# hypermagik/srsRAN-5G

Measured on AMD Instinct MI355X. Metric: PDSCH+PUSCH slots/sec (100MHz 4x4) + LDPC info-bits/s at 1/2/4/8 GPU, higher is better.
Workload: dtype int8/bf16/f32; 1 GPU

## Files before the change

srsran-5g_amd/csrc/capi_pdsch_mod.cpp:

```cpp
#include "capi_internal.h"
#include <algorithm>
#include <cmath>
#include <cstring>
#include <vector>

using namespace srsgpu;

static_assert(sizeof(srsgpu_pdsch_mod_config) == 168, "srsgpu_pdsch_mod_config layout (mirrored by srsgpu.PdschModConfig)");

static_assert(sizeof(srsgpu_pdsch_dmrs_config) == 152, "srsgpu_pdsch_dmrs_config layout (mirrored by srsgpu)");

struct srsgpu_pdsch_dmrs_plan {
  srsgpu_context* ctx      = nullptr;
  device_buffer<dmrs_job> d_jobs;
  device_buffer<uint32_t> d_seq;
  int             nof_jobs = 0;
  int             max_pilots = 0;
};

struct srsgpu_pdsch_modulator_plan {
  srsgpu_context* ctx        = nullptr;
  device_buffer<mod_desc>  d_desc;
  device_buffer<uint16_t>  d_sc_map;
  device_buffer<float>     d_prg_w;
// ... 216 lines not shown
    if (c.nof_symbols < 1 || c.start_symbol + c.nof_symbols > 14) {
      return fail(SRSGPU_ERR_INVALID_ARG, "tx %u: time allocation [%u, %u) exceeds the slot", t, c.start_symbol,
                  c.start_symbol + c.nof_symbols);
    }
    if ((c.dmrs_type != 1 && c.dmrs_type != 2) || c.nof_cdm_groups_without_data < 1 ||
        c.nof_cdm_groups_without_data > (c.dmrs_type == 1 ? 2 : 3)) {
      return fail(SRSGPU_ERR_INVALID_ARG, "tx %u: invalid DM-RS type %u / CDM groups without data %u", t,
                  c.dmrs_type, c.nof_cdm_groups_without_data);
    }
    const bool general = x != nullptr && (x->crb_mask != nullptr || x->nof_reserved > 0 || x->prg_size > 0);
    if (c.n_id > 1023 || c.bwp_size_rb < 1 || c.bwp_start_rb + c.bwp_size_rb > grid_nof_prb ||
        (!general && (c.nof_rb < 1 || c.rb_start + c.nof_rb > c.bwp_size_rb))) {
      return fail(SRSGPU_ERR_INVALID_ARG, "tx %u: allocation outside the BWP or the grid, or n_id > 1023", t);
    }
    if (x != nullptr && ((x->nof_reserved > 0 && x->reserved == nullptr) ||
                         (x->prg_size > 0 && (x->prg_weights == nullptr || x->nof_prg == 0 ||
                                              static_cast<uint32_t>(x->prg_size) * x->nof_prg < grid_nof_prb)))) {
      return fail(SRSGPU_ERR_INVALID_ARG, "tx %u: invalid allocation extension (reserved patterns / PRG weights)", t);
    }
    if (c.cw_offset % 4 != 0) {
      return fail(SRSGPU_ERR_INVALID_ARG, "tx %u: codeword offset not a multiple of 4", t);
    }
    mod_desc d{};
    unsigned nd = 0;
    for (unsigned k = 0; k < 12; ++k) {
      const unsigned group = (c.dmrs_type == 2) ? (k % 6) / 2 : k % 2;
      if (group >= c.nof_cdm_groups_without_data) {
        d.dmrs_lut |= static_cast<uint64_t>(k) << (4 * nd);
        ++nd;
      }
    }
    d.nd_dmrs = static_cast<uint8_t>(nd);
    uint32_t nre = 0;
    d.sc_map     = NO_SC_MAP;
    if (general) {
      std::vector<uint8_t> crbs(grid_nof_prb, 0);
      for (unsigned rb = 0; rb < grid_nof_prb; ++rb) {
        crbs[rb] = (x->crb_mask != nullptr) ? x->crb_mask[rb]
                                            : (rb >= c.bwp_start_rb + c.rb_start &&
                                               rb < static_cast<unsigned>(c.bwp_start_rb + c.rb_start + c.nof_rb));
      }
      enumerate_data_res(grid_nof_prb, crbs.data(), c.start_symbol, c.nof_symbols, c.dmrs_symbol_mask, c.dmrs_type,
                         c.nof_cdm_groups_without_data, c.bwp_start_rb, c.bwp_start_rb + c.bwp_size_rb, x->reserved,
                         x->nof_reserved, sc_tx, d.sym_cum);
      nre      = static_cast<uint32_t>(sc_tx.size());
      d.sc_map = static_cast<uint32_t>(sc_map.size());
      sc_map.insert(sc_map.end(), sc_tx.begin(), sc_tx.end());
    } else {
      for (unsigned l = 0; l < 14; ++l) {
        d.sym_cum[l] = static_cast<uint16_t>(nre);
        if (l >= c.start_symbol && l < static_cast<unsigned>(c.start_symbol + c.nof_symbols)) {
          nre += (((c.dmrs_symbol_mask >> l) & 1u) ? nd : 12u) * c.nof_rb;
        }
      }
      d.sym_cum[14] = static_cast<uint16_t>(nre);
      d.sym_cum[15] = static_cast<uint16_t>(nre);
    }
    const uint64_t need = static_cast<uint64_t>(nre) * c.nof_layers * qm;
    if (nre == 0 || need != c.nof_bits || c.nof_bits > MOD_MAX_BITS) {
      return fail(SRSGPU_ERR_INVALID_ARG, "tx %u: codeword of %u bits for %u data REs x %u layers x Qm %u", t,
                  c.nof_bits, nre, c.nof_layers, qm);
    }
    d.cw_word_offset = c.cw_offset / 4;
    d.nof_bits       = c.nof_bits;
    d.c_init         = (static_cast<uint32_t>(c.rnti) << 15) + c.n_id;
    d.port_stride    = 14u * nsc;
    d.nsc            = nsc;
    d.grid_base      = c.grid_index * grid_nof_ports * 14u * nsc + (general ? 0u : (c.bwp_start_rb + c.rb_start) * 12u);
    d.dmrs_mask      = c.dmrs_symbol_mask;
    d.qm             = static_cast<uint8_t>(qm);
    d.L              = c.nof_layers;
    d.P              = c.nof_ports;
    float amp = modulation_amplitude(qm);
    if (std::isnormal(c.scaling)) {
      amp *= c.scaling;
    }
    for (int p = 0; p < 4; ++p) {
      for (int l = 0; l < 4; ++l) {
        const bool used = p < c.nof_ports && l < c.nof_layers;
        d.w[p][l][0]    = used ? c.precoding[p][l][0] * amp : 0.f;
        d.w[p][l][1]    = used ? c.precoding[p][l][1] * amp : 0.f;
      }
    }
    d.prg_sc = 0;
    if (x != nullptr && x->prg_size > 0) {
      d.prg_sc = static_cast<uint16_t>(x->prg_size * 12u);
      d.prg_w  = static_cast<uint32_t>(prg_w.size());
      for (unsigned g = 0; g < x->nof_prg; ++g) {
        for (int p = 0; p < 4; ++p) {
          for (int l = 0; l < 4; ++l) {
            const bool   used = p < c.nof_ports && l < c.nof_layers;
            const float* src  = x->prg_weights + ((static_cast<size_t>(g) * c.nof_ports + p) * c.nof_layers + l) * 2;
            prg_w.push_back(used ? src[0] * amp : 0.f);
            prg_w.push_back(used ? src[1] * amp : 0.f);
          }
        }
      }
    }
    descs[t]              = d;
    const uint32_t Lq     = static_cast<uint32_t>(c.nof_layers) * qm;
    const uint32_t nwords = (c.nof_bits + 31) / 32;
    for (uint32_t w0 = 0; w0 < nwords; w0 += MOD_CHUNK_WORDS) {
      const uint32_t b0 = w0 * 32, b1 = b0 + MOD_CHUNK_WORDS * 32;
      mod_chunk      ch{};
      ch.tx       = t;
      ch.word0    = w0;
      ch.re_begin = (b0 + Lq - 1) / Lq;
      ch.re_end   = std::min(nre, (b1 + Lq - 1) / Lq);
      if (ch.re_end > ch.re_begin) {
        chunks.push_back(ch);
      }
    }
  }
  std::vector<uint32_t> c_inits(descs.size()), nwords(descs.size());
  for (size_t t = 0; t < descs.size(); ++t) {
    c_inits[t] = descs[t].c_init;
    nwords[t]  = (descs[t].nof_bits + 31u) / 32u;
  }
  const std::vector<uint32_t> seq_off = gold_sequence_offsets(nwords);
  for (size_t t = 0; t < descs.size(); ++t) {
    descs[t].seq_word_offset = seq_off[t];
  }
  plan_ptr<srsgpu_pdsch_modulator_plan> plan(new srsgpu_pdsch_modulator_plan());
  plan->ctx        = ctx;
  plan->nof_chunks = static_cast<int>(chunks.size());
  if (!chunks.empty()) {
    if (build_gold_sequences(ctx, c_inits, nwords, seq_off, plan->d_seq) != SRSGPU_OK) {
      return SRSGPU_ERR_HIP;
    }
    if (!plan->d_desc.upload(descs) || !plan->d_chunks.upload(chunks) || !plan->d_sc_map.upload(sc_map) ||
        !plan->d_prg_w.upload(prg_w)) {
      return fail(SRSGPU_ERR_HIP, "failed to upload modulator descriptors");
    }
  }
  *plan_out = plan.release();
  return SRSGPU_OK;
}

int srsgpu_pdsch_modulator_plan_execute(const srsgpu_pdsch_modulator_plan* plan,
                                        const uint8_t*                     d_codewords,
                                        uint32_t*                          d_grids,
                                        void*                              stream)
{
  if (plan == nullptr || d_codewords == nullptr || d_grids == nullptr) {
    return fail(SRSGPU_ERR_INVALID_ARG, "null argument");
  }
  launch_pdsch_modulate(plan->d_desc.get(), plan->d_sc_map.get(), plan->d_prg_w.get(), plan->d_chunks.get(),
                        plan->nof_chunks, reinterpret_cast<const uint32_t*>(d_codewords), d_grids, plan->d_seq.get(),
                        static_cast<hipStream_t>(stream));
  HIP_TRY(hipGetLastError());
  return SRSGPU_OK;
}

void srsgpu_pdsch_modulator_plan_destroy(srsgpu_pdsch_modulator_plan* plan)
{
  if (plan == nullptr) {
    return;
  }
  delete plan;
}

int srsgpu_pdsch_dmrs_plan_create(srsgpu_context*                 ctx,
                                  const srsgpu_pdsch_dmrs_config* cfgs,
                                  uint32_t                        nof_tx,
                                  uint32_t                        grid_nof_prb,
                                  uint32_t                        grid_nof_ports,
                                  srsgpu_pdsch_dmrs_plan**        plan_out)
{
// ... 132 lines not shown
```

srsran-5g_amd/csrc/crc_device.h:

```cpp
#pragma once

#include "common.h"

namespace srsgpu {

__device__ __forceinline__ uint32_t gf2_mulmod(uint32_t a, uint32_t b, uint32_t g, int order)
{
  const uint32_t high = 1u << order;
  uint32_t       r    = 0;
  for (int i = order - 1; i >= 0; --i) {
    r <<= 1;
    if (r & high) {
      r ^= g;
    }
    if ((b >> i) & 1u) {
      r ^= a;
    }
  }
  return r;
}

__device__ inline uint32_t block_crc_bytes(const uint8_t* data, int n, int order, uint32_t g, uint32_t* table,
                                           uint32_t* part)
{
// ... 24 lines not shown
  }
  __syncthreads();
  uint32_t f = 1u;
  {
    uint32_t base = 2u;
    uint32_t e    = 8u * static_cast<uint32_t>(cs);
    while (e) {
      if (e & 1u) {
        f = gf2_mulmod(f, base, g, order);
      }
      base = gf2_mulmod(base, base, g, order);
      e >>= 1;
    }
  }
  for (int step = 1; step < 256; step <<= 1) {
    if (in && (threadIdx.x % (2 * step)) == 0) {
      part[threadIdx.x] = gf2_mulmod(part[threadIdx.x], f, g, order) ^ part[threadIdx.x + step];
    }
    f = gf2_mulmod(f, f, g, order);
    __syncthreads();
  }
  const uint32_t crc = part[0];
  __syncthreads();
  return crc;
}

__device__ inline uint32_t block_crc_table(const uint8_t* data, int nbytes, const uint32_t* P, uint32_t* red)
{
  uint32_t acc = 0;
  for (int j = threadIdx.x; j < nbytes; j += blockDim.x) {
    const uint32_t byte = data[j];
    const uint4*   p4   = reinterpret_cast<const uint4*>(P + 8 * j);
    const uint4    a    = p4[0];
    const uint4    b    = p4[1];
    acc ^= (byte & 0x80u) ? a.x : 0u;
    acc ^= (byte & 0x40u) ? a.y : 0u;
    acc ^= (byte & 0x20u) ? a.z : 0u;
    acc ^= (byte & 0x10u) ? a.w : 0u;
    acc ^= (byte & 0x08u) ? b.x : 0u;
    acc ^= (byte & 0x04u) ? b.y : 0u;
    acc ^= (byte & 0x02u) ? b.z : 0u;
    acc ^= (byte & 0x01u) ? b.w : 0u;
  }
  acc = wave_xor(acc);
  if ((threadIdx.x % WAVE) == 0) {
    red[threadIdx.x / WAVE] = acc;
  }
  __syncthreads();
  uint32_t crc = 0;
  for (int w = 0; w < static_cast<int>(blockDim.x / WAVE); ++w) {
    crc ^= red[w];
  }
  __syncthreads();
  return crc;
}

__device__ inline void crc_byte_lut(uint32_t* lut, int order, uint32_t g)
{
  const uint32_t mask = (1u << order) - 1u;
  for (uint32_t t = threadIdx.x; t < 256u; t += blockDim.x) {
    uint32_t r = t << (order - 8);
    for (int k = 0; k < 8; ++k) {
      r <<= 1;
      if (r & (1u << order)) {
        r ^= g;
      }
    }
    lut[t] = r & mask;
  }
  __syncthreads();
}

__device__ __forceinline__ uint32_t gf2_mulmod(uint32_t r, uint32_t M, int order, uint32_t g)
{
  uint32_t acc = 0;
#pragma unroll
  for (int b = 23; b >= 0; --b) {
    acc = (acc << 1) ^ (((acc >> (order - 1)) & 1u) ? g : 0u);
    acc ^= ((M >> b) & 1u) ? r : 0u;
  }
  return acc;
}

__device__ __forceinline__ uint32_t crc_step4(uint32_t r, uint32_t m, int order, const uint32_t* T)
{
  const uint32_t u = (r << (32 - order)) ^ m;
  return T[u & 0xffu] ^ T[256u + ((u >> 8) & 0xffu)] ^ T[512u + ((u >> 16) & 0xffu)] ^ T[768u + (u >> 24)];
}

template <int CS, typename Data>
__device__ inline uint32_t block_crc_slice4(Data data, int nbytes, const uint32_t* P, int order, uint32_t g,
                                            const uint32_t* T, uint32_t* red, bool have_m0 = false, uint32_t m0 = 0)
{
  static_assert(CS % 4 == 0, "whole words per chunk");
  const uint32_t mask = (1u << order) - 1u;
  const int      L    = 8 * nbytes;
  const int      nch  = (nbytes + CS - 1) / CS;
  const int      c0   = static_cast<int>(threadIdx.x);
  uint32_t       acc  = 0;
  for (int c = c0; c < nch; c += blockDim.x) {
    const int      b0 = c * CS;
    const int      b1 = min(b0 + CS, nbytes);
    const int      j  = 8 * b1 + order - 1;
    const uint32_t M  = (have_m0 && c == c0) ? m0 : ((j < L) ? P[j] : (1u << (order + L - 1 - j)));
    uint32_t       byte[CS];
#pragma unroll
    for (int k = 0; k < CS; ++k) {
      byte[k] = (b0 + k < b1) ? static_cast<uint32_t>(data(b0 + k)) : 0u;
    }
    uint32_t rem = 0;
#pragma unroll
    for (int w = 0; w < CS / 4; ++w) {
      const int k = 4 * w;
      if (b0 + k + 4 <= b1) {
        rem = crc_step4(rem, (byte[k] << 24) | (byte[k + 1] << 16) | (byte[k + 2] << 8) | byte[k + 3], order, T);
      } else {
#pragma unroll
        for (int q = 0; q < 4; ++q) {
          if (b0 + k + q < b1) {
            rem = ((rem << 8) ^ T[((rem >> (order - 8)) ^ byte[k + q]) & 0xffu]) & mask;
          }
        }
      }
    }
    acc ^= gf2_mulmod(rem, M, order, g);
  }
  acc = wave_xor(acc);
  if ((threadIdx.x % WAVE) == 0) {
    red[threadIdx.x / WAVE] = acc;
  }
  __syncthreads();
  uint32_t crc = 0;
  for (int w = 0; w < static_cast<int>((blockDim.x + WAVE - 1) / WAVE); ++w) {
    crc ^= red[w];
  }
  __syncthreads();
  return crc;
}

template <int CS>
__device__ __forceinline__ uint32_t crc_chunk_power(int c, int nbytes, const uint32_t* P, int order)
{
  const int L  = 8 * nbytes;
  const int b1 = min((c + 1) * CS, nbytes);
  const int j  = 8 * b1 + order - 1;
  return (j < L) ? P[j] : (1u << (order + L - 1 - j));
}

template <int CS, typename Data>
__device__ inline uint32_t block_crc_chunks(Data data, int nbytes, const uint32_t* P, int order, uint32_t g,
                                            const uint32_t* lut, uint32_t* red, int begin = 0, int end = -1,
                                            bool have_m0 = false, uint32_t m0 = 0)
{
  const uint32_t mask = (1u << order) - 1u;
  const int      L    = 8 * nbytes;
  const int      nch  = ((end < 0 ? nbytes : end) + CS - 1) / CS;
  const int      c0   = begin / CS + static_cast<int>(threadIdx.x);
  uint32_t       acc  = 0;
  for (int c = c0; c < nch; c += blockDim.x) {
    const int b0  = c * CS;
    const int b1  = min(b0 + CS, nbytes);
    const int j   = 8 * b1 + order - 1;
    const uint32_t M = (have_m0 && c == c0) ? m0 : ((j < L) ? P[j] : (1u << (order + L - 1 - j)));
    uint32_t byte[CS];
#pragma unroll
    for (int k = 0; k < CS; ++k) {
      byte[k] = (b0 + k < b1) ? static_cast<uint32_t>(data(b0 + k)) : 0u;
    }
    uint32_t rem = 0;
#pragma unroll
    for (int k = 0; k < CS; ++k) {
      if (b0 + k < b1) {
        rem = ((rem << 8) ^ lut[((rem >> (order - 8)) ^ byte[k]) & 0xffu]) & mask;
      }
    }
    acc ^= gf2_mulmod(rem, M, order, g);
  }
  acc = wave_xor(acc);
  if ((threadIdx.x % WAVE) == 0) {
    red[threadIdx.x / WAVE] = acc;
  }
  __syncthreads();
  uint32_t crc = 0;
  for (int w = 0; w < static_cast<int>((blockDim.x + WAVE - 1) / WAVE); ++w) {
    crc ^= red[w];
  }
  __syncthreads();
  return crc;
}

}
```

srsran-5g_amd/csrc/ldpc_encoder.hip:

```cpp
#include "common.h"
#include "crc_device.h"
#include "ldpc_base_graphs.h"
#include "srsgpu_internal.h"

namespace srsgpu {
namespace {

#ifdef ENC_PROFILE
constexpr int ENC_PROF_CBS   = 8192;
constexpr int ENC_PROF_SLOTS = 16;
__device__ uint64_t g_enc_prof[ENC_PROF_CBS * ENC_PROF_SLOTS];
#define ENC_PROF(slot, value)                                                                                          \
  do {                                                                                                                 \
    if (threadIdx.x == 0 && blockIdx.x < ENC_PROF_CBS) {                                                               \
      g_enc_prof[blockIdx.x * ENC_PROF_SLOTS + (slot)] = (value);                                                      \
    }                                                                                                                  \
  } while (0)
#else
#define ENC_PROF(slot, value)                                                                                          \
  do {                                                                                                                 \
  } while (0)
#endif
#define ENC_STAMP(slot) ENC_PROF(slot, __builtin_amdgcn_s_memtime())

// ... 493 lines not shown
  tcd.order       = d.tb_crc_len;
  tcd.poly        = (d.tb_crc_len == 24) ? 0x1864cfbu : 0x11021u;
  tcd.table       = d.tb_crc_table;
  constexpr int TCS   = 16;
  const bool    tfast = carrier && tcd.nbytes <= 2u * TCS * PK_THREADS && ((tcd.byte_offset | tcd.nbytes) & 3u) == 0u;
  uint32_t      tw[2][TCS / 4];
  uint32_t      tm[2] = {0u, 0u};
  if (tfast) {
    const uint32_t* tbw = reinterpret_cast<const uint32_t*>(tbs + tcd.byte_offset);
    const int       nw  = static_cast<int>(tcd.nbytes / 4u);
#pragma unroll
    for (int h = 0; h < 2; ++h) {
      const int c = tid + h * PK_THREADS;
#pragma unroll
      for (int q = 0; q < TCS / 4; ++q) {
        const int w = c * (TCS / 4) + q;
        tw[h][q]    = (w < nw) ? tbw[w] : 0u;
      }
      if (c * TCS < static_cast<int>(tcd.nbytes)) {
        tm[h] = crc_chunk_power<TCS>(c, static_cast<int>(tcd.nbytes), crc_tables + tcd.table,
                                     static_cast<int>(tcd.order));
      }
    }
  }
  constexpr int TW = CRC_SLICE_WORDS / PK_THREADS;
  if (has_cbc) {
    const uint32_t* src = crc_slice + CRC_SLICE_24B * CRC_SLICE_WORDS;
    uint32_t        t[TW];
#pragma unroll
    for (int q = 0; q < TW; ++q) {
      t[q] = src[tid + q * PK_THREADS];
    }
#pragma unroll
    for (int q = 0; q < TW; ++q) {
      t4b[tid + q * PK_THREADS] = t[q];
    }
  }
  if (carrier) {
    const uint32_t* src = crc_slice + (tcd.order == 24 ? CRC_SLICE_24A : CRC_SLICE_16) * CRC_SLICE_WORDS;
    uint32_t        t[TW];
#pragma unroll
    for (int q = 0; q < TW; ++q) {
      t[q] = src[tid + q * PK_THREADS];
    }
#pragma unroll
    for (int q = 0; q < TW; ++q) {
      uni[tid + q * PK_THREADS] = t[q];
    }
  }
  for (int m = tid; m <= G::M; m += PK_THREADS) {
    row_start[m] = static_cast<uint16_t>(G::rs(m));
  }
#pragma unroll
  for (int r = 0; r < MB; ++r) {
    const int q = tid + r * PK_THREADS;
    if (q < nkb) {
      const uint32_t p = d.tb_bit_offset + 8u * static_cast<uint32_t>(q);
      uint32_t       b = byte[r];
      if (q < nd8 && p >= d.tb_bits) {
        b = (tb_crc >> (d.tb_crc_len - 8u - (p - d.tb_bits))) & 0xffu;
      }
      msg[q] = static_cast<uint8_t>(b);
    }
  }
  __syncthreads();
  if (tfast) {
    const int order  = static_cast<int>(tcd.order);
    const int nb     = static_cast<int>(tcd.nbytes);
    uint32_t  rem[2] = {0u, 0u};
#pragma unroll
    for (int q = 0; q < TCS / 4; ++q) {
#pragma unroll
      for (int h = 0; h < 2; ++h) {
        const int c = tid + h * PK_THREADS;
        if (c * TCS + 4 * q < nb) {
          rem[h] = crc_step4(rem[h], __builtin_bswap32(tw[h][q]), order, t4t);
        }
      }
    }
    uint32_t acc = 0;
#pragma unroll
    for (int h = 0; h < 2; ++h) {
      if ((tid + h * PK_THREADS) * TCS < nb) {
        acc ^= gf2_mulmod(rem[h], tm[h], order, tcd.poly);
      }
    }
    acc = wave_xor(acc);
    if ((tid % WAVE) == 0) {
      red[tid / WAVE] = acc;
    }
    __syncthreads();
#pragma unroll
    for (int w = 0; w < PK_THREADS / WAVE; ++w) {
      tb_crc ^= red[w];
    }
  } else if (carrier) {
    const uint8_t* tbp = tbs + tcd.byte_offset;
    tb_crc = block_crc_slice4<16>([tbp](int i) { return tbp[i]; }, static_cast<int>(tcd.nbytes),
                                  crc_tables + tcd.table, static_cast<int>(tcd.order), tcd.poly, t4t, red);
  }
  ENC_STAMP(1);
  if (carrier) {
    const int qc = static_cast<int>(d.tb_bits - min(d.tb_bit_offset, d.tb_bits)) / 8;
    if (tid < nd8 - qc) {
      const uint32_t p = d.tb_bit_offset + 8u * static_cast<uint32_t>(qc + tid);
      msg[qc + tid]    = static_cast<uint8_t>((tb_crc >> (d.tb_crc_len - 8u - (p - d.tb_bits))) & 0xffu);
    }
  }
  ENC_STAMP(2);
  if (has_cbc) {
    if (carrier) {
      __syncthreads();
    }
    const uint32_t crc = block_crc_slice4<CB_CS>([](int q) { return msg[q]; }, cb_bytes, crc_tables + d.crc_table, 24,
                                                 0x1800063u, t4b, red, pre_m, m0);
    if (tid < 3) {
      msg[d.used / 8 + tid] = static_cast<uint8_t>(crc >> (16 - 8 * tid));
    }
  }
  __syncthreads();
  ENC_STAMP(3);
  const uint32_t* msg32 = reinterpret_cast<const uint32_t*>(msg);
  for (int q = tid; q < K * W; q += PK_THREADS) {
    cw[q] = bytes_bitrev(msg32[q]);
  }
  if (tid < 4 * WMAX) {
    lam[tid] = 0u;
  }
#pragma unroll
  for (int r = 0; r < NEL; ++r) {
    if (tid + r * PK_THREADS < G::NE) {
      edge[tid + r * PK_THREADS] = ev[r];
    }
  }
  __syncthreads();
  ENC_STAMP(4);
  {
    const int CH     = (W <= 10) ? 3 : 2;
    const int ntask  = 4 * W * CH;
    if (tid < ntask) {
      const int m     = tid / (W * CH);
      const int rem   = tid - m * W * CH;
      const int ch    = rem / W;
      const int k     = rem - ch * W;
      const int rs    = row_start[m];
      const int deg   = row_start[m + 1] - rs;
      const int per   = (deg + CH - 1) / CH;
      const int e_beg = rs + ch * per;
      const int e_end = min(e_beg + per, rs + deg);
      constexpr int MAXCH = (core_max_degree<BG>() + 1) / 2;
      uint32_t acc = 0;
#pragma unroll
      for (int q = 0; q < MAXCH; ++q) {
        const int e = e_beg + q;
        if (e < e_end) {
          const uint32_t ce = edge[e];
          const int      c  = static_cast<int>(ce >> 16);
          if (c < K) {
            acc ^= col_window(cw + c * W, k, static_cast<int>(ce & 0xffffu), W);
          }
        }
      }
      if (acc != 0u) {
        atomicXor(&lam[m * WMAX + k], acc);
      }
    }
  }
  __syncthreads();
  ENC_STAMP(5);
  if (tid < WAVE) {
    const core_plan cp = core_plans[d.zpos];
    if (tid < W) {
      const int k   = tid;
      const int o   = cp.o0;
      cw[K * W + k] = col_window(lam, k, o, W) ^ col_window(lam + WMAX, k, o, W) ^
                      col_window(lam + 2 * WMAX, k, o, W) ^ col_window(lam + 3 * WMAX, k, o, W);
    }
#pragma unroll
    for (int step = 0; step < 3; ++step) {
      __builtin_amdgcn_fence(__ATOMIC_RELEASE, "workgroup");
      __builtin_amdgcn_wave_barrier();
      __builtin_amdgcn_fence(__ATOMIC_ACQUIRE, "workgroup");
      if (tid < W) {
        const int k   = tid;
        uint32_t  acc = col_window(lam + cp.row[step] * WMAX, k, cp.orow[step], W);
#pragma unroll
        for (int j = 0; j < 4; ++j) {
          const int oj = cp.oj[step][j];
          if (oj >= 0) {
            acc ^= col_window(cw + (K + j) * W, k, oj, W);
          }
        }
        cw[(K + cp.unk[step]) * W + k] = acc;
      }
    }
  }
  __syncthreads();
  ENC_STAMP(6);
// ... 100 lines not shown
```

srsran-5g_amd/csrc/pdsch_modulator.hip:

```cpp
#include "gold_device.h"
#include "signal_device.h"
#include "srsgpu_internal.h"

#pragma clang fp contract(off)

namespace srsgpu {
namespace {

constexpr int MOD_THREADS = 256;

__device__ __forceinline__ uint32_t scrambled_word(const mod_desc& d,
                                                   const uint32_t* __restrict__ cw,
                                                   const uint32_t* __restrict__ seq,
                                                   uint32_t w)
{
  return __builtin_bswap32(*reinterpret_cast<const uint32_t*>(reinterpret_cast<const char*>(cw) +
                                                              (d.cw_word_offset + w) * 4u)) ^
         *reinterpret_cast<const uint32_t*>(reinterpret_cast<const char*>(seq) + (d.seq_word_offset + w) * 4u);
}

__global__ __launch_bounds__(MOD_THREADS) void gold_fill_kernel(const uint32_t* __restrict__ c_inits,
                                                                 const uint32_t* __restrict__ offsets,
                                                                 const uint32_t* __restrict__ nwords,
                                                                 const uint32_t* __restrict__ wstart,
                                                                 uint32_t* __restrict__ seq,
                                                                 const uint32_t* __restrict__ x1,
                                                                 const uint32_t* __restrict__ x2_jump,
                                                                 const uint32_t* __restrict__ x2_lane)
{
  const uint32_t t = blockIdx.y;
  const uint32_t i = blockIdx.x * MOD_THREADS + threadIdx.x;
  if (i < nwords[t]) {
    const uint32_t w = (wstart != nullptr ? wstart[t] : 0u) + i;
    seq[offsets[t] + i] = gold_word(c_inits[t], w, w >> 6, x1, x2_jump, x2_lane);
  }
}

__device__ __forceinline__ float2 constellation_point(uint32_t idx, uint32_t qm)
{
  int re = 0, im = 0, off = -1;
  for (uint32_t j = 0; j < qm / 2; ++j) {
    re += off;
    im += off;
    off *= 2;
    re = ((idx >> (2 * j + 1)) & 1u) ? re : -re;
    im = ((idx >> (2 * j)) & 1u) ? im : -im;
  }
  return make_float2(static_cast<float>(re), static_cast<float>(im));
}

template <bool MAP, bool PRG>
__device__ __forceinline__ void modulate_res(const mod_desc& d,
                                             const mod_chunk& ch,
                                             const uint32_t*  bits,
                                             const float2*    points,
                                             const uint16_t* __restrict__ sc_map,
                                             const float* __restrict__ prg_w,
                                             uint32_t* __restrict__ grids)
{
  const uint32_t tid = threadIdx.x;
  const uint32_t qm = d.qm, L = d.L, P = d.P, Lq = L * qm;
  const uint32_t qmask = (1u << qm) - 1u;
  float          w[4][4][2];
#pragma unroll
  for (int p = 0; p < 4; ++p) {
#pragma unroll
    for (int l = 0; l < 4; ++l) {
      w[p][l][0] = d.w[p][l][0];
      w[p][l][1] = d.w[p][l][1];
    }
  }

  uint32_t l = 0, next = 0;
  for (uint32_t r = ch.re_begin + tid; r < ch.re_end; r += MOD_THREADS) {
    const uint32_t o  = r * Lq - ch.word0 * 32u;
    const uint32_t wi = o >> 5;
    const uint64_t b  = ((static_cast<uint64_t>(bits[wi]) << 32) | bits[wi + 1]) << (o & 31u);

    if (r >= next) {
      l    = 0;
      next = 0xffffffffu;
#pragma unroll
      for (int j = 1; j < 15; ++j) {
        const uint32_t c = d.sym_cum[j];
        l += (c <= r) ? 1u : 0u;
        next = (c > r && c < next) ? c : next;
      }
    }
    const uint32_t k = r - d.sym_cum[l];
    uint32_t       sc;
    if constexpr (MAP) {
      sc = sc_map[d.sc_map + r];
    } else if ((d.dmrs_mask >> l) & 1u) {
      const uint32_t nd  = d.nd_dmrs;
      const uint32_t prb = k / nd;
      const uint32_t j   = k - prb * nd;
      sc                 = prb * 12u + static_cast<uint32_t>((d.dmrs_lut >> (4u * j)) & 15u);
    } else {
      sc = k;
    }
    const uint32_t e = d.grid_base + l * d.nsc + sc;
    const float* wt = PRG ? prg_w + d.prg_w + (sc / d.prg_sc) * 32u : nullptr;

    float xr[4], xi[4];
#pragma unroll
    for (int ly = 0; ly < 4; ++ly) {
      if (ly < static_cast<int>(L)) {
        const float2 x = points[static_cast<uint32_t>(b >> (64u - (ly + 1) * qm)) & qmask];
        xr[ly]         = x.x;
        xi[ly]         = x.y;
      }
    }

#pragma unroll
    for (int p = 0; p < 4; ++p) {
      if (p < static_cast<int>(P)) {
        float sr = 0.f, si = 0.f;
#pragma unroll
        for (int ly = 0; ly < 4; ++ly) {
          if (ly < static_cast<int>(L)) {
            const float wr = PRG ? wt[(p * 4 + ly) * 2] : w[p][ly][0];
            const float wi = PRG ? wt[(p * 4 + ly) * 2 + 1] : w[p][ly][1];
            const float pr = xr[ly] * wr - xi[ly] * wi;
            const float pi = xr[ly] * wi + xi[ly] * wr;
            sr             = (ly == 0) ? pr : sr + pr;
            si             = (ly == 0) ? pi : si + pi;
          }
        }
        *reinterpret_cast<uint32_t*>(reinterpret_cast<char*>(grids) + (e + static_cast<uint32_t>(p) * d.port_stride) * 4u) =
            bf16_bits(sr) | (bf16_bits(si) << 16);
      }
    }
  }
}

__global__ __launch_bounds__(MOD_THREADS) void pdsch_modulate_kernel(const mod_desc* __restrict__ descs,
                                                                      const uint16_t* __restrict__ sc_map,
                                                                      const float* __restrict__ prg_w,
                                                                      const mod_chunk* __restrict__ chunks,
                                                                      const uint32_t* __restrict__ cw,
                                                                      uint32_t* __restrict__ grids,
                                                                      const uint32_t* __restrict__ seq)
{
  __shared__ uint32_t bits[MOD_CHUNK_WORDS + 1];
  __shared__ float2   points[256];
  const mod_chunk ch  = chunks[blockIdx.x];
  const mod_desc& d   = descs[ch.tx];
  const uint32_t  tid = threadIdx.x;
  const uint32_t  nwords = (d.nof_bits + 31u) >> 5;
  static_assert(MOD_THREADS >= 256, "one constellation point per lane");
  if (tid < (1u << d.qm)) {
    points[tid] = constellation_point(tid, d.qm);
  }

  for (uint32_t j = tid; j < MOD_CHUNK_WORDS; j += MOD_THREADS) {
    const uint32_t w = ch.word0 + j;
    bits[j]          = (w < nwords) ? scrambled_word(d, cw, seq, w) : 0u;
  }
  {
    if (tid == 0) {
      const uint32_t w2 = ch.word0 + MOD_CHUNK_WORDS;
      bits[MOD_CHUNK_WORDS] = (w2 < nwords) ? scrambled_word(d, cw, seq, w2) : 0u;
    }
  }

  __syncthreads();
  if (d.sc_map == NO_SC_MAP) {
    modulate_res<false, false>(d, ch, bits, points, sc_map, prg_w, grids);
  } else if (d.prg_sc == 0) {
    modulate_res<true, false>(d, ch, bits, points, sc_map, prg_w, grids);
  } else {
    modulate_res<true, true>(d, ch, bits, points, sc_map, prg_w, grids);
  }
}

__global__ __launch_bounds__(MOD_THREADS) void pdsch_dmrs_kernel(const dmrs_job* __restrict__ jobs,
                                                                  uint32_t* __restrict__ grids,
                                                                  const uint32_t* __restrict__ gseq)
{
  const dmrs_job& jb     = jobs[blockIdx.x];
  const uint32_t  per_rb = jb.type2 ? 4u : 6u;
  const uint32_t  wfirst = (2 * jb.seq_offset) >> 5;
  for (uint32_t i = threadIdx.x + blockIdx.y * blockDim.x; i < jb.nof_pilots; i += blockDim.x * gridDim.y) {
    const uint32_t n    = 2 * (jb.seq_offset + i);
    const uint32_t w    = n >> 5;
    const uint32_t word = gseq[jb.gseq_base + (w - wfirst)];
    const uint32_t sh   = 31u - (n & 31u);
    const float    re   = ((word >> sh) & 1u) ? -jb.amp : jb.amp;
    const float    im   = ((word >> (sh - 1)) & 1u) ? -jb.amp : jb.amp;
    const uint32_t rb   = i / per_rb, j = i - rb * per_rb;
    for (uint32_t g = 0; 2 * g < jb.L; ++g) {
      const uint32_t k = rb * 12u + (jb.type2 ? 6u * (j >> 1) + 2u * g + (j & 1u) : 2u * j + g);
      const float s1 = (i & 1u) ? -1.f : 1.f;
      const uint32_t q0 = 2 * g, q1 = 2 * g + 1;
#pragma unroll
      for (int p = 0; p < 4; ++p) {
        if (p < static_cast<int>(jb.P)) {
          const float wr0 = jb.w[p][q0][0], wi0 = jb.w[p][q0][1];
          float       sr  = re * wr0 - im * wi0;
          float       si  = re * wi0 + im * wr0;
          if (q1 < jb.L) {
            const float a = re * s1, b = im * s1;
            const float wr1 = jb.w[p][q1][0], wi1 = jb.w[p][q1][1];
            sr = sr + (a * wr1 - b * wi1);
            si = si + (a * wi1 + b * wr1);
          }
          grids[jb.grid_base + static_cast<uint32_t>(p) * jb.port_stride + k] =
              bf16_bits(sr) | (bf16_bits(si) << 16);
        }
      }
    }
  }
}

}

void launch_pdsch_dmrs(const dmrs_job* d_jobs,
                       int             nof_jobs,
                       int             max_pilots,
                       uint32_t*       d_grids,
                       const uint32_t* d_seq,
                       hipStream_t     stream)
{
  if (nof_jobs <= 0) {
    return;
  }
  const int      threads = max_pilots <= 64 ? 64 : MOD_THREADS;
  const unsigned ny      = static_cast<unsigned>((max_pilots + threads - 1) / threads);
  hipLaunchKernelGGL(pdsch_dmrs_kernel, dim3(static_cast<unsigned>(nof_jobs), ny > 0 ? ny : 1u),
                     dim3(static_cast<unsigned>(threads)), 0,
                     stream, d_jobs, d_grids, d_seq);
}

void launch_pdsch_modulate(const mod_desc*  d_desc,
                           const uint16_t*  d_sc_map,
                           const float*     d_prg_w,
                           const mod_chunk* d_chunks,
                           int              nof_chunks,
                           const uint32_t*  d_codewords,
                           uint32_t*        d_grids,
                           const uint32_t*  d_seq,
                           hipStream_t      stream)
{
  if (nof_chunks <= 0) {
    return;
  }
  hipLaunchKernelGGL(pdsch_modulate_kernel, dim3(static_cast<unsigned>(nof_chunks)), dim3(MOD_THREADS), 0, stream,
                     d_desc, d_sc_map, d_prg_w, d_chunks, d_codewords, d_grids, d_seq);
}

void launch_gold_fill(const uint32_t* d_c_inits,
                      const uint32_t* d_offsets,
                      const uint32_t* d_nwords,
// ... 19 lines not shown
```

srsran-5g_amd/csrc/srsgpu_internal.h:

```cpp
#pragma once

#include <hip/hip_runtime.h>
#include <cstdint>

#include "srsgpu_phy.h"

namespace srsgpu {

constexpr int SOFT_COL_STRIDE = 384;

constexpr uint32_t NO_CRC_TABLE = 0xffffffffu;

struct dec_desc {
  uint32_t llr_offset;
  uint32_t nof_llr;
  uint32_t out_offset;
  uint32_t crc_table;
  uint32_t div_magic;
  uint16_t Z;
  uint16_t zpos;
  uint16_t nof_significant;
  uint16_t max_iter;
  uint32_t sf16;
  float    sf;
// ... 151 lines not shown
                            uint8_t*           d_tb_crc_ok,
                            const uint32_t*    d_crc_tables,
                            uint32_t*          d_acc,
                            uint32_t*          d_cnt,
                            hipStream_t        stream);

void launch_pusch_tb(const tb_dec_desc* d_desc,
                     int                nof_tbs,
                     int                threads,
                     uint8_t*           d_cb_crc_ok,
                     const uint8_t*     d_cb_msgs,
                     uint8_t*           d_tbs,
                     uint8_t*           d_tb_crc_ok,
                     const uint32_t*    d_crc_tables,
                     hipStream_t        stream);

constexpr uint32_t CB_MSG_STRIDE = 1056;

#ifdef CHEST_PROFILE
int debug_read_chest_profile(uint64_t* dst, size_t n);
#endif
#ifdef ENC_PROFILE
int debug_read_encoder_profile(uint64_t* dst, size_t n);
#endif
#ifdef LDPC_DEC_PROFILE
constexpr int LDPC_DEC_PROF_CBS   = 4096;
constexpr int LDPC_DEC_PROF_SLOTS = 32;
int debug_read_decoder_profile(uint64_t* dst, size_t n);
int debug_read_decoder_profile_pk(uint64_t* dst, size_t n);
#endif

struct dec_group {
  int       bg         = 1;
  bool      packed     = false;
  int       max_layers = 0;
  int       split      = 1;
  int       pack       = 1;
  int       threads    = 64;
  int       count      = 0;
  dec_desc* d_desc     = nullptr;
  dm_desc*  d_dm       = nullptr;
};

struct dec_launch_args {
  int             mode         = 1;
  const int8_t*   d_llrs       = nullptr;
  const int8_t*   d_cw_llrs    = nullptr;
  uint8_t*        d_out        = nullptr;
  int32_t*        d_results    = nullptr;
  const uint32_t* d_crc_tables = nullptr;
  uint8_t*        d_cb_crc_ok  = nullptr;
  int8_t*         d_harq       = nullptr;
  int8_t* const*  d_harq_cbs   = nullptr;
  uint8_t*        d_tbs        = nullptr;
  uint8_t*        d_tb_crc_ok  = nullptr;
  hipStream_t     stream       = nullptr;
};

void launch_ldpc_decode_pk(const dec_group& g, const uint32_t* d_ab, const dec_launch_args& a);

void launch_ldpc_decode_pairs(const dec_group& g, const uint32_t* d_ab2, const dec_launch_args& a);

void launch_ldpc_decode(const dec_group& g, const uint32_t* d_shifts, const dec_launch_args& a);

struct mod_desc {
  uint64_t dmrs_lut;
  uint32_t cw_word_offset;
  uint32_t nof_bits;
  uint32_t c_init;
  uint32_t grid_base;
  uint32_t port_stride;
  uint32_t nsc;
  uint16_t dmrs_mask;
  uint8_t  qm;
  uint8_t  L;
  uint8_t  P;
  uint8_t  nd_dmrs;
  uint16_t prg_sc;
  uint16_t sym_cum[16];
  float    w[4][4][2];
  uint32_t seq_word_offset;
  uint32_t sc_map;
  uint32_t prg_w;
  uint32_t pad3[3];
};
static_assert(sizeof(mod_desc) == 224, "mod_desc layout");

constexpr uint32_t NO_SC_MAP = 0xffffffffu;

struct mod_chunk {
  uint32_t tx;
  uint32_t word0;
  uint32_t re_begin;
  uint32_t re_end;
};

constexpr uint32_t MOD_CHUNK_WORDS = 1024;
constexpr uint32_t DEMOD_CHUNK_WORDS = 256;
constexpr uint32_t MOD_MAX_BITS    = 1u << 21;
constexpr uint32_t GOLD_NC           = 1600;
constexpr uint32_t GOLD_X1_WORDS     = MOD_MAX_BITS / 32;
constexpr uint32_t GOLD_X2_JUMPS     = MOD_MAX_BITS / 2048;

void launch_pdsch_modulate(const mod_desc*  d_desc,
                           const uint16_t*  d_sc_map,
                           const float*     d_prg_w,
                           const mod_chunk* d_chunks,
                           int              nof_chunks,
                           const uint32_t*  d_codewords,
                           uint32_t*        d_grids,
                           const uint32_t*  d_seq,
                           hipStream_t      stream);

void launch_gold_fill(const uint32_t* d_c_inits,
                      const uint32_t* d_offsets,
                      const uint32_t* d_nwords,
                      const uint32_t* d_wstart,
                      int             nof_tx,
                      uint32_t        max_nwords,
                      uint32_t*       d_seq,
                      const uint32_t* d_x1,
                      const uint32_t* d_x2_jump,
                      const uint32_t* d_x2_lane,
                      hipStream_t     stream);

struct ofdm_job {
  uint32_t grid_offset;
  uint32_t sample_offset;
  uint32_t cp_len;
  uint32_t pad;
  float    coef_re;
  float    coef_im;
};

constexpr uint32_t OFDM_MAX_DFT = 8192;

constexpr uint32_t ofdm_split_factor(uint32_t n)
{
  return n == 9216 ? 9 : n == 12288 ? 3 : n == 18432 ? 9 : n == 24576 ? 3 : n == 36864 ? 9 : n == 49152 ? 6
         : n == 98304 ? 12 : 0;
}

void launch_ofdm(bool            inverse,
                 uint32_t        dft_size,
                 const ofdm_job* d_jobs,
                 int             nof_jobs,
                 uint32_t        nsc,
                 uint32_t        window_offset,
                 const float*    d_twiddles,
                 const uint32_t* d_grid_in,
                 uint32_t*       d_grid_out,
                 const float*    d_samples_in,
                 float*          d_samples_out,
                 float*          d_scratch,
                 hipStream_t     stream,
                 const uint32_t* d_twin = nullptr);
bool launch_ofdm_direct(bool                          inverse,
                        uint32_t                      dft_size,
                        const srsgpu_ofdm_direct_job* d_jobs,
                        int                           nof_jobs,
                        uint32_t                      nsc,
                        uint32_t                      window_offset,
                        const float*                  d_twiddles,
                        hipStream_t                   stream);

struct demod_desc {
  uint64_t dmrs_lut;
  uint32_t grid_base;
  uint32_t port_stride;
// ... 358 lines not shown
```

Before: 173,500 slots/s.

## Skip zero precoding weights in modulator and speed up CRC combine and word loads

The host now builds a sparsity mask of the nonzero precoding weights, and the modulator kernel dispatches to specialised variants (dense, identity-4x4, masked) that skip multiplications by zero weights. Separately, the CRC chunk combine replaces a 24-step bitwise GF(2) multiply with a byte-table-assisted version. The code-block CRC also reads whole 32-bit words from shared memory instead of individual bytes. These changes aim to cut ALU work in the modulation and the LDPC encoder CRC, at the cost of more template instantiations and larger code.

Result: faster. 177,900 slots/s, median of 6 (+2.5%).

```diff
diff --git a/srsran-5g_amd/csrc/capi_pdsch_mod.cpp b/srsran-5g_amd/csrc/capi_pdsch_mod.cpp
--- a/srsran-5g_amd/csrc/capi_pdsch_mod.cpp
+++ b/srsran-5g_amd/csrc/capi_pdsch_mod.cpp
@@ -322,8 +322,23 @@
         d.w[p][l][1]    = used ? c.precoding[p][l][1] * amp : 0.f;
       }
     }
+    uint32_t w_mask   = 0;
+    bool     zero_row = false;
+    for (int p = 0; p < c.nof_ports; ++p) {
+      uint32_t row = 0;
+      for (int l = 0; l < c.nof_layers; ++l) {
+        if (!(d.w[p][l][0] == 0.f && d.w[p][l][1] == 0.f)) {
+          row |= 1u << (p * 4 + l);
+        }
+      }
+      zero_row = zero_row || row == 0;
+      w_mask |= row;
+    }
+    const bool no_zeros = __builtin_popcount(w_mask) == c.nof_ports * c.nof_layers;
+    d.w_mask            = (zero_row || no_zeros) ? MOD_W_MASK_DENSE : w_mask;
     d.prg_sc = 0;
     if (x != nullptr && x->prg_size > 0) {
+      d.w_mask = MOD_W_MASK_DENSE;
       d.prg_sc = static_cast<uint16_t>(x->prg_size * 12u);
       d.prg_w  = static_cast<uint32_t>(prg_w.size());
       for (unsigned g = 0; g < x->nof_prg; ++g) {
diff --git a/srsran-5g_amd/csrc/crc_device.h b/srsran-5g_amd/csrc/crc_device.h
--- a/srsran-5g_amd/csrc/crc_device.h
+++ b/srsran-5g_amd/csrc/crc_device.h
@@ -130,6 +130,22 @@
   return acc;
 }
 
+__device__ __forceinline__ uint32_t gf2_mulmod_bytes(uint32_t r, uint32_t M, int order, const uint32_t* T0)
+{
+  const uint32_t mask = (1u << order) - 1u;
+  const uint32_t M8   = ((M << 8) & mask) ^ T0[M >> (order - 8)];
+  const uint32_t M16  = ((M8 << 8) & mask) ^ T0[M8 >> (order - 8)];
+  uint32_t       acc  = 0;
+#pragma unroll
+  for (int b = 7; b >= 0; --b) {
+    const uint32_t s0 = static_cast<uint32_t>(static_cast<int32_t>(r << (31 - b)) >> 31);
+    const uint32_t s1 = static_cast<uint32_t>(static_cast<int32_t>(r << (23 - b)) >> 31);
+    const uint32_t s2 = static_cast<uint32_t>(static_cast<int32_t>(r << (15 - b)) >> 31);
+    acc               = (acc << 1) ^ (s0 & M) ^ (s1 & M8) ^ (s2 & M16);
+  }
+  return (acc & mask) ^ T0[acc >> order];
+}
+
 __device__ __forceinline__ uint32_t crc_step4(uint32_t r, uint32_t m, int order, const uint32_t* T)
 {
   const uint32_t u = (r << (32 - order)) ^ m;
@@ -137,8 +153,9 @@
 }
 
 template <int CS, typename Data>
-__device__ inline uint32_t block_crc_slice4(Data data, int nbytes, const uint32_t* P, int order, uint32_t g,
-                                            const uint32_t* T, uint32_t* red, bool have_m0 = false, uint32_t m0 = 0)
+__device__ inline uint32_t block_crc_slice4(Data data, int nbytes, const uint32_t* P, int order, const uint32_t* T,
+                                            uint32_t* red, bool have_m0 = false, uint32_t m0 = 0,
+                                            const uint32_t* words = nullptr)
 {
   static_assert(CS % 4 == 0, "whole words per chunk");
   const uint32_t mask = (1u << order) - 1u;
@@ -151,27 +168,39 @@
     const int      b1 = min(b0 + CS, nbytes);
     const int      j  = 8 * b1 + order - 1;
     const uint32_t M  = (have_m0 && c == c0) ? m0 : ((j < L) ? P[j] : (1u << (order + L - 1 - j)));
-    uint32_t       byte[CS];
-#pragma unroll
-    for (int k = 0; k < CS; ++k) {
-      byte[k] = (b0 + k < b1) ? static_cast<uint32_t>(data(b0 + k)) : 0u;
-    }
-    uint32_t rem = 0;
-#pragma unroll
-    for (int w = 0; w < CS / 4; ++w) {
-      const int k = 4 * w;
-      if (b0 + k + 4 <= b1) {
-        rem = crc_step4(rem, (byte[k] << 24) | (byte[k + 1] << 16) | (byte[k + 2] << 8) | byte[k + 3], order, T);
-      } else {
-#pragma unroll
-        for (int q = 0; q < 4; ++q) {
-          if (b0 + k + q < b1) {
-            rem = ((rem << 8) ^ T[((rem >> (order - 8)) ^ byte[k + q]) & 0xffu]) & mask;
+    uint32_t       rem = 0;
+    if (words != nullptr && b0 + CS <= b1) {
+      uint32_t word[CS / 4];
+#pragma unroll
+      for (int w = 0; w < CS / 4; ++w) {
+        word[w] = words[b0 / 4 + w];
+      }
+#pragma unroll
+      for (int w = 0; w < CS / 4; ++w) {
+        rem = crc_step4(rem, __builtin_bswap32(word[w]), order, T);
+      }
+    } else {
+      uint32_t byte[CS];
+#pragma unroll
+      for (int k = 0; k < CS; ++k) {
+        byte[k] = (b0 + k < b1) ? static_cast<uint32_t>(data(b0 + k)) : 0u;
+      }
+#pragma unroll
+      for (int w = 0; w < CS / 4; ++w) {
+        const int k = 4 * w;
+        if (b0 + k + 4 <= b1) {
+          rem = crc_step4(rem, (byte[k] << 24) | (byte[k + 1] << 16) | (byte[k + 2] << 8) | byte[k + 3], order, T);
+        } else {
+#pragma unroll
+          for (int q = 0; q < 4; ++q) {
+            if (b0 + k + q < b1) {
+              rem = ((rem << 8) ^ T[((rem >> (order - 8)) ^ byte[k + q]) & 0xffu]) & mask;
+            }
           }
         }
       }
     }
-    acc ^= gf2_mulmod(rem, M, order, g);
+    acc ^= gf2_mulmod_bytes(rem, M, order, T);
   }
   acc = wave_xor(acc);
   if ((threadIdx.x % WAVE) == 0) {
diff --git a/srsran-5g_amd/csrc/ldpc_encoder.hip b/srsran-5g_amd/csrc/ldpc_encoder.hip
--- a/srsran-5g_amd/csrc/ldpc_encoder.hip
+++ b/srsran-5g_amd/csrc/ldpc_encoder.hip
@@ -599,7 +599,7 @@
 #pragma unroll
     for (int h = 0; h < 2; ++h) {
       if ((tid + h * PK_THREADS) * TCS < nb) {
-        acc ^= gf2_mulmod(rem[h], tm[h], order, tcd.poly);
+        acc ^= gf2_mulmod_bytes(rem[h], tm[h], order, t4t);
       }
     }
     acc = wave_xor(acc);
@@ -614,7 +614,7 @@
   } else if (carrier) {
     const uint8_t* tbp = tbs + tcd.byte_offset;
     tb_crc = block_crc_slice4<16>([tbp](int i) { return tbp[i]; }, static_cast<int>(tcd.nbytes),
-                                  crc_tables + tcd.table, static_cast<int>(tcd.order), tcd.poly, t4t, red);
+                                  crc_tables + tcd.table, static_cast<int>(tcd.order), t4t, red);
   }
   ENC_STAMP(1);
   if (carrier) {
@@ -630,7 +630,7 @@
       __syncthreads();
     }
     const uint32_t crc = block_crc_slice4<CB_CS>([](int q) { return msg[q]; }, cb_bytes, crc_tables + d.crc_table, 24,
-                                                 0x1800063u, t4b, red, pre_m, m0);
+                                                 t4b, red, pre_m, m0, reinterpret_cast<const uint32_t*>(msg));
     if (tid < 3) {
       msg[d.used / 8 + tid] = static_cast<uint8_t>(crc >> (16 - 8 * tid));
     }
diff --git a/srsran-5g_amd/csrc/pdsch_modulator.hip b/srsran-5g_amd/csrc/pdsch_modulator.hip
--- a/srsran-5g_amd/csrc/pdsch_modulator.hip
+++ b/srsran-5g_amd/csrc/pdsch_modulator.hip
@@ -49,7 +49,9 @@
   return make_float2(static_cast<float>(re), static_cast<float>(im));
 }
 
-template <bool MAP, bool PRG>
+enum { W_DENSE = 0, W_MASK = 1, W_IDENTITY4 = 2 };
+
+template <bool MAP, bool PRG, int SPARSE = W_DENSE>
 __device__ __forceinline__ void modulate_res(const mod_desc& d,
                                              const mod_chunk& ch,
                                              const uint32_t*  bits,
@@ -59,7 +61,9 @@
                                              uint32_t* __restrict__ grids)
 {
   const uint32_t tid = threadIdx.x;
-  const uint32_t qm = d.qm, L = d.L, P = d.P, Lq = L * qm;
+  static_assert(!PRG || SPARSE == W_DENSE, "the mask describes the wideband weights");
+  const uint32_t qm = d.qm, L = (SPARSE == W_IDENTITY4) ? 4u : d.L, P = (SPARSE == W_IDENTITY4) ? 4u : d.P, Lq = L * qm;
+  const uint32_t wmask = (SPARSE == W_IDENTITY4) ? MOD_W_MASK_IDENTITY4 : d.w_mask;
   const uint32_t qmask = (1u << qm) - 1u;
   float          w[4][4][2];
 #pragma unroll
@@ -116,15 +120,22 @@
     for (int p = 0; p < 4; ++p) {
       if (p < static_cast<int>(P)) {
         float sr = 0.f, si = 0.f;
+        bool  first = true;
 #pragma unroll
         for (int ly = 0; ly < 4; ++ly) {
-          if (ly < static_cast<int>(L)) {
+          if (ly < static_cast<int>(L) && (SPARSE == W_DENSE || ((wmask >> (p * 4 + ly)) & 1u) != 0)) {
             const float wr = PRG ? wt[(p * 4 + ly) * 2] : w[p][ly][0];
             const float wi = PRG ? wt[(p * 4 + ly) * 2 + 1] : w[p][ly][1];
             const float pr = xr[ly] * wr - xi[ly] * wi;
             const float pi = xr[ly] * wi + xi[ly] * wr;
-            sr             = (ly == 0) ? pr : sr + pr;
-            si             = (ly == 0) ? pi : si + pi;
+            if constexpr (SPARSE == W_DENSE) {
+              sr = (ly == 0) ? pr : sr + pr;
+              si = (ly == 0) ? pi : si + pi;
+            } else {
+              sr    = first ? pr : sr + pr;
+              si    = first ? pi : si + pi;
+              first = false;
+            }
           }
         }
         *reinterpret_cast<uint32_t*>(reinterpret_cast<char*>(grids) + (e + static_cast<uint32_t>(p) * d.port_stride) * 4u) =
@@ -165,10 +176,23 @@
   }
 
   __syncthreads();
+  const uint32_t wmask = __builtin_amdgcn_readfirstlane(d.w_mask);
   if (d.sc_map == NO_SC_MAP) {
-    modulate_res<false, false>(d, ch, bits, points, sc_map, prg_w, grids);
+    if (wmask == MOD_W_MASK_DENSE) {
+      modulate_res<false, false>(d, ch, bits, points, sc_map, prg_w, grids);
+    } else if (wmask == MOD_W_MASK_IDENTITY4) {
+      modulate_res<false, false, W_IDENTITY4>(d, ch, bits, points, sc_map, prg_w, grids);
+    } else {
+      modulate_res<false, false, W_MASK>(d, ch, bits, points, sc_map, prg_w, grids);
+    }
   } else if (d.prg_sc == 0) {
-    modulate_res<true, false>(d, ch, bits, points, sc_map, prg_w, grids);
+    if (wmask == MOD_W_MASK_DENSE) {
+      modulate_res<true, false>(d, ch, bits, points, sc_map, prg_w, grids);
+    } else if (wmask == MOD_W_MASK_IDENTITY4) {
+      modulate_res<true, false, W_IDENTITY4>(d, ch, bits, points, sc_map, prg_w, grids);
+    } else {
+      modulate_res<true, false, W_MASK>(d, ch, bits, points, sc_map, prg_w, grids);
+    }
   } else {
     modulate_res<true, true>(d, ch, bits, points, sc_map, prg_w, grids);
   }
diff --git a/srsran-5g_amd/csrc/srsgpu_internal.h b/srsran-5g_amd/csrc/srsgpu_internal.h
--- a/srsran-5g_amd/csrc/srsgpu_internal.h
+++ b/srsran-5g_amd/csrc/srsgpu_internal.h
@@ -257,9 +257,13 @@
   uint32_t seq_word_offset;
   uint32_t sc_map;
   uint32_t prg_w;
-  uint32_t pad3[3];
+  uint32_t w_mask;
+  uint32_t pad3[2];
 };
 static_assert(sizeof(mod_desc) == 224, "mod_desc layout");
+
+constexpr uint32_t MOD_W_MASK_DENSE = 0u;
+constexpr uint32_t MOD_W_MASK_IDENTITY4 = 0x8421u;
 
 constexpr uint32_t NO_SC_MAP = 0xffffffffu;
 
```
